# JulHoltzDevelopers/WavesAndEigenvalues.jl

Hardware: AMD Instinct MI355X
Metric: eigenpairs/sec (higher is better)
Workload: dtype f64

## Files before the change

### wavesandeigenvalues.jl_amd/csrc/beyn.hip

```cpp
#include <cmath>

#include "solver.h"

static void small_solve(std::vector<zc> &A, std::vector<zc> &b, int n) {
    std::vector<char> dead(n, 0);
    double amax = 0.0;
    for (const zc &a : A) amax = std::max(amax, std::abs(a));
    for (int k = 0; k < n; ++k) {
        int p = k;
        double best = 0.0;
        for (int i = k; i < n; ++i) { const double v = std::abs(A[(size_t)k * n + i]); if (v > best) { best = v; p = i; } }
        if (!(best > 1e-14 * amax)) { dead[k] = 1; continue; }
        if (p != k) {
            for (int j = 0; j < n; ++j) std::swap(A[(size_t)j * n + k], A[(size_t)j * n + p]);
            std::swap(b[k], b[p]);
        }
        const zc inv = 1.0 / A[(size_t)k * n + k];
        for (int i = k + 1; i < n; ++i) {
            const zc f = A[(size_t)k * n + i] * inv;
            if (f == zc(0)) continue;
            for (int j = k + 1; j < n; ++j) A[(size_t)j * n + i] -= f * A[(size_t)j * n + k];
            b[i] -= f * b[k];
        }
    }
    for (int k = n - 1; k >= 0; --k) {
        if (dead[k]) { b[k] = 0; continue; }
        zc sres = b[k];
        for (int j = k + 1; j < n; ++j) sres -= A[(size_t)j * n + k] * b[j];
        b[k] = sres / A[(size_t)k * n + k];
    }
}

static void rb_d2h(wae_family *h, const cplx *src, cplx *dst, size_t cnt) {
    HIP_CHECK(hipMemcpyAsync(dst, src, cnt * sizeof(cplx), hipMemcpyDeviceToHost, h->stream));
    HIP_CHECK(hipStreamSynchronize(h->stream));
}

static void rb_reset(wae_family *h, cplx *Q, int cap, int l, const double *table, int npts, const cplx *Vinter) {
    RbState &R = h->rb;
    const int T = h->T;
    R.Q = Q; R.cap = cap; R.l = l; R.S = 0;
    R.kact.clear();
    for (int k = 0; k < T; ++k) {
        bool used = false;
        for (int p = 0; p < npts && !used; ++p) used = table[((size_t)p * T + k) * 2] != 0.0 || table[((size_t)p * T + k) * 2 + 1] != 0.0;
        if (used) R.kact.push_back(k);
    }
    const size_t vecl = (size_t)h->d * l;
    R.wait_w();
    if (R.W.n < R.kact.size() * (size_t)cap * vecl) {
        const size_t need = R.kact.size() * (size_t)cap * vecl;
        const int dev = h->device;
        RbState *Rp = &R;
        R.w_job = std::async(std::launch::async, [Rp, need, dev]() {
            HIP_CHECK(hipSetDevice(dev));
            Rp->W.alloc(need);
        });
    }
    R.Hk.assign(R.kact.size() * (size_t)cap * cap * l, zc(0));
    R.g.assign((size_t)cap * l, zc(0));
    R.Vi.reserve(vecl);
    HIP_CHECK(hipMemcpyAsync(R.Vi.p, Vinter, vecl * sizeof(cplx), hipMemcpyDeviceToDevice, h->stream));
    R.vi_valid = true;
    R.hb.reserve((size_t)4 * (cap + 4) * l); R.alpha.reserve(l); R.alpha2.reserve((size_t)cap * l);
}

static void rb_append_block(wae_family *h, int cnt, const std::vector<std::vector<std::vector<zc>>> &pck) {
    RbState &R = h->rb;
    hipStream_t st = h->stream;
    const int64_t d = h->d;
    const int l = R.l, cap = R.cap, S = R.S;
    const size_t vecl = (size_t)d * l;
    std::vector<cplx> hh((size_t)(S + cnt) * cnt * l), n0((size_t)cnt * l), n1(l);
    const OpDev A0 = h->ops[0].dev(WAE_OP_N);
    cplx *qn = R.Q + (size_t)S * vecl;
    for (int j = 0; j < cnt; ++j) launch_norms(qn + (size_t)j * vecl, d, l, h->partial.p, R.hb.p + (size_t)j * l, st);
    rb_d2h(h, R.hb.p, n0.data(), (size_t)cnt * l);
    static const bool multi_axpy = !(getenv("WAE_RB_MULTI_AXPY") && atoi(getenv("WAE_RB_MULTI_AXPY")) == 0);
    const bool fits = (size_t)S * cnt * l * sizeof(cplx) <= 60 * 1024;
    for (int pass = 0; pass < 2 && S > 0; ++pass) {
        launch_dots_multi(R.Q, vecl, S, qn, vecl, cnt, d, l, h->partial.p, R.hb.p, st);
        if (multi_axpy && fits) {
            launch_axpy_neg_multi(R.Q, vecl, S, R.hb.p, qn, vecl, cnt, d, l, st);
            continue;
        }
        rb_d2h(h, R.hb.p, hh.data(), (size_t)S * cnt * l);
        std::vector<cplx> cj((size_t)S * l);
        for (int j = 0; j < cnt; ++j) {
            for (int i = 0; i < S; ++i)
                for (int c = 0; c < l; ++c) cj[(size_t)i * l + c] = hh[((size_t)i * cnt + j) * l + c];
            R.alpha2.upload(cj.data(), cj.size(), st);
            launch_axpy_neg(R.Q, vecl, S, R.alpha2.p, qn + (size_t)j * vecl, d, l, st);
            HIP_CHECK(hipStreamSynchronize(st));
        }
    }
    for (int j = 0; j < cnt; ++j) {
        cplx *q = qn + (size_t)j * vecl;
        for (int pass = 0; pass < 2 && j > 0; ++pass) {
            launch_dots(qn, vecl, j, q, d, l, h->partial.p, R.hb.p, st);
            launch_axpy_neg(qn, vecl, j, R.hb.p, q, d, l, st);
        }
        launch_norms(q, d, l, h->partial.p, R.hb.p, st);
        rb_d2h(h, R.hb.p, n1.data(), l);
        for (int c = 0; c < l; ++c) {
            const double nrm0 = n0[(size_t)j * l + c].x;
            n1[c] = (n1[c].x > 1e-9 * nrm0 && nrm0 > 0.0) ? cplx{n1[c].x, 0.0} : cplx{0.0, 0.0};
        }
        R.alpha.upload(n1.data(), l, st);
        launch_scale_inv(q, R.alpha.p, q, d, l, st);
        HIP_CHECK(hipStreamSynchronize(st));
    }
    launch_dots_multi(qn, vecl, cnt, R.Vi.p, vecl, 1, d, l, h->partial.p, R.hb.p, st);
    rb_d2h(h, R.hb.p, hh.data(), (size_t)cnt * l);
    for (int j = 0; j < cnt; ++j)
        for (int c = 0; c < l; ++c) R.g[(size_t)(S + j) * l + c] = zc(hh[(size_t)j * l + c].x, hh[(size_t)j * l + c].y);
    for (size_t ki = 0; ki < R.kact.size(); ++ki) {
        R.wait_w();
        cplx *Wk = R.W.p + ki * (size_t)cap * vecl;
        cplx *wn = Wk + (size_t)S * vecl;
        upload_pc(h, pck[ki]);
        for (int j = 0; j < cnt; ++j)
            launch_spmv(A0, pc_level(h, 0), l, qn + (size_t)j * vecl, wn + (size_t)j * vecl, nullptr, 0.0, l, MODE_AX, st);
        zc *H = &R.Hk[ki * (size_t)cap * cap * l];
        launch_dots_multi(R.Q, vecl, S + cnt, wn, vecl, cnt, d, l, h->partial.p, R.hb.p, st);
        rb_d2h(h, R.hb.p, hh.data(), (size_t)(S + cnt) * cnt * l);
        for (int i = 0; i < S + cnt; ++i)
            for (int j = 0; j < cnt; ++j)
                for (int c = 0; c < l; ++c) {
                    const cplx v = hh[((size_t)i * cnt + j) * l + c];
                    H[((size_t)(S + j) * cap + i) * l + c] = zc(v.x, v.y);
                }
        zc herm_factor(0);
        bool herm = false;
        {
            static const bool herm_on = !(getenv("WAE_RB_HERMITIAN") && atoi(getenv("WAE_RB_HERMITIAN")) == 0);
            const int kterm = R.kact[ki], pl = h->term_plane[kterm];
            const LevelOp &L0 = h->ops[0];
            for (size_t g = 0; g < L0.groups.size() && herm_on && !herm; ++g)
                for (int q = 0; q < L0.groups[g].nplanes; ++q)
                    if (h->slot_plane[0][(size_t)L0.groups[g].plane0 + q] == pl && L0.groups[g].symmetric && L0.groups[g].is_real) {
                        const zc sc = h->term_scale[kterm];
                        if (sc != zc(0)) { herm = true; herm_factor = sc / std::conj(sc); }
                    }
        }
        if (S > 0 && herm) {
            for (int i = 0; i < S; ++i)
                for (int j = 0; j < cnt; ++j)
                    for (int c = 0; c < l; ++c)
                        H[((size_t)i * cap + S + j) * l + c] = herm_factor * std::conj(H[((size_t)(S + j) * cap + i) * l + c]);
        } else if (S > 0) {
            launch_dots_multi(Wk, vecl, S, qn, vecl, cnt, d, l, h->partial.p, R.hb.p, st);
            rb_d2h(h, R.hb.p, hh.data(), (size_t)S * cnt * l);
            for (int i = 0; i < S; ++i)
                for (int j = 0; j < cnt; ++j)
                    for (int c = 0; c < l; ++c) {
                        const cplx v = hh[((size_t)i * cnt + j) * l + c];
                        H[((size_t)i * cap + S + j) * l + c] = zc(v.x, -v.y);
                    }
        }
    }
    R.S += cnt;
}

static void rb_append(wae_family *h, int count) {
    RbState &R = h->rb;
    WAE_REQUIRE(R.S + count <= R.cap, "snapshot store is full");
    std::vector<std::vector<std::vector<zc>>> pck(R.kact.size());
    for (size_t ki = 0; ki < R.kact.size(); ++ki) {
        std::vector<double> ek((size_t)2 * h->T, 0.0);
        ek[(size_t)2 * R.kact[ki]] = 1.0;
        pck[ki].resize(1);
        plane_coeffs(h, ek.data(), WAE_OP_N, pck[ki][0]);
    }
    for (int done = 0; done < count; done += 4) rb_append_block(h, std::min(4, count - done), pck);
}

static std::vector<cplx> rb_guess_coeffs(const wae_family *h, const double *ct_chunk, int ns) {
    const RbState &R = h->rb;
    const int S = R.S, l = R.l, cap = R.cap, T = h->T, nb = ns * l;
    std::vector<cplx> Y((size_t)S * nb);
    std::vector<zc> Hs((size_t)S * S), rhs(S);
    for (int sy = 0; sy < ns; ++sy) {
        const double *ct = ct_chunk + (size_t)sy * 2 * T;
        for (int k = 0; k < T; ++k)
            if ((ct[2 * k] != 0.0 || ct[2 * k + 1] != 0.0) && std::find(R.kact.begin(), R.kact.end(), k) == R.kact.end())
                throw WaeError(WAE_ERR_INVALID, "a term outside the projected set has a non-zero coefficient: rebuild the basis (mode 1)");
        for (int c = 0; c < l; ++c) {
            std::fill(Hs.begin(), Hs.end(), zc(0));
            for (size_t ki = 0; ki < R.kact.size(); ++ki) {
                const zc ck(ct[2 * R.kact[ki]], ct[2 * R.kact[ki] + 1]);
                if (ck == zc(0)) continue;
                const zc *H = &R.Hk[ki * (size_t)cap * cap * l];
                for (int sc = 0; sc < S; ++sc)
                    for (int i = 0; i < S; ++i) Hs[(size_t)sc * S + i] += ck * H[((size_t)sc * cap + i) * l + c];
            }
            for (int i = 0; i < S; ++i) rhs[i] = R.g[(size_t)i * l + c];
            small_solve(Hs, rhs, S);
            for (int i = 0; i < S; ++i) {
                const zc yv = std::isfinite(rhs[i].real()) && std::isfinite(rhs[i].imag()) ? rhs[i] : zc(0);
                Y[(size_t)i * nb + (size_t)sy * l + c] = cplx{yv.real(), yv.imag()};
            }
        }
    }
    return Y;
}
static void rb_apply_guess(wae_family *h, const std::vector<cplx> &Y, int ns, cplx *X) {
    RbState &R = h->rb;
    const int S = (int)(Y.size() / ((size_t)ns * R.l));
    R.ycoef.upload(Y.data(), Y.size(), h->stream);
    launch_lincomb_rep(R.Q, (size_t)h->d * R.l, S, R.ycoef.p, X, h->d, ns * R.l, R.l, h->stream);
    HIP_CHECK(hipStreamSynchronize(h->stream));
}

struct BeynPass {
    enum Keep { nothing, into_basis, raw_to_store };
    bool new_basis = false;
    int absorb = 0;
    bool solve = true;
    bool guess = false;
    Keep keep = nothing;
    int enrich_its = 1 << 30;
    bool light_cycle = false;
    bool progressive = false;
    bool prefetch_coeffs = false;
    int npts = 0;
    const double *z = nullptr, *w = nullptr, *coeff_table = nullptr;
    const double *V = nullptr;
    int l = 0, l_total = 0, col0 = 0;
    int K = 1, maxit = 0;
    double tol = 0.0;
    cplx *Q = nullptr;
    int nbasis = 0, slot0 = 0;
    double *A_out = nullptr;
    cplx *out_dev = nullptr;
    bool accumulate = false;
};

static BeynPass beyn_pass_for_mode(int mode, bool have_V, int npts, int nbasis, int slot0) {
    WAE_REQUIRE(have_V || mode == 2, "bad argument");
    WAE_REQUIRE(mode >= 0 && mode <= 4, "mode must be 0 (take snapshots), 1 (rebuild the basis from the store, use it), 2 (use it), "
                                        "3 (solve from zero, store raw) or 4 (build the basis from the store, solve nothing)");
    WAE_REQUIRE(nbasis >= 0 && slot0 >= 0 && (mode == 2 || slot0 + ((mode == 0 || mode == 3) ? npts : 0) <= nbasis), "snapshot slots out of range");
    static const int enrich_its = getenv("WAE_RB_ENRICH") ? atoi(getenv("WAE_RB_ENRICH")) : (1 << 30);
    BeynPass p;
// ... 40 lines not shown
    const bool store = p.new_basis || p.guess || p.keep != BeynPass::nothing;
    WAE_REQUIRE(!store || p.l <= h->NB, "l exceeds the solver batch width");
    HIP_CHECK(hipSetDevice(h->device));
    hipStream_t st = h->stream;
    CallInfo ci;
    const int64_t d = h->d;
    const int l = p.l, T = h->T, npts = p.npts, npow = 2 * p.K;
    const size_t acnt = (size_t)d * p.l_total * npow;
    const size_t vecl = (size_t)d * l;
    RbState &R = h->rb;
    DevBuf<cplx> Aown;
    cplx *Ad = p.out_dev;
    if (!Ad) { Aown.alloc(acnt); Ad = Aown.p; }
    if (!p.accumulate) launch_fill_zero(Ad, acnt, st);
    cplx *Q = p.Q;
    if (store && !Q) {
        if (p.new_basis && p.keep == BeynPass::into_basis) h->rbQ.reserve(vecl * (size_t)p.nbasis);
        WAE_REQUIRE(h->rbQ.n >= vecl * (size_t)p.nbasis, "no snapshots stored in the handle: run mode 0 first");
        Q = h->rbQ.p;
    }
    h->io_a.reserve(vecl);
    if (p.V) {
        HIP_CHECK(hipMemcpyAsync(h->io_a.p, p.V, vecl * sizeof(cplx), hipMemcpyHostToDevice, st));
    } else {
        WAE_REQUIRE(R.vi_valid && R.l == l && R.Vi.n >= vecl, "V may be NULL only in mode 2 after a mode 0/1 call with the same l on this handle");
        launch_inter_to_colmajor(R.Vi.p, l, d, l, h->io_a.p, st, h->perm());
    }
    if (p.guess) R.ycoef.reserve((size_t)std::max(p.nbasis, 1) * h->NB);
    if (p.new_basis) {
        launch_colmajor_to_inter(h->io_a.p, d, l, h->W.p, l, st, h->perm());
        rb_reset(h, Q, p.nbasis, l, p.coeff_table, npts, h->W.p);
        if (p.absorb > 0) rb_append(h, p.absorb);
    } else if (p.guess) {
        WAE_REQUIRE(R.Q == Q && R.l == l && R.cap == p.nbasis, "the basis in the handle belongs to another store / shape");
        WAE_REQUIRE(p.keep != BeynPass::into_basis || p.slot0 == R.S, "mode 0 appends: slot0 must equal the number of snapshots taken so far");
        WAE_REQUIRE(p.keep == BeynPass::into_basis || R.S > 0, "mode 2 needs a basis: run mode 0 (or 1) first");
    }
    if (!p.solve) {
        HIP_CHECK(hipStreamSynchronize(st));
        ci.li.levels = (int)h->ops.size();
        return ci.finish(info);
    }

    static const bool rbdbg = getenv("WAE_GMRES_DEBUG") && atoi(getenv("WAE_GMRES_DEBUG"));
    double t_guess = 0.0, t_solve = 0.0, t_append = 0.0;
    struct LightOff { bool &on; ~LightOff() { on = false; } } light_off{h->vc_light};
    for (int cg = 0; cg < l; cg += h->NB) {
        const int lg = std::min(h->NB, l - cg);
        const int spc = std::max(1, h->NB / lg);
        const int c0 = std::max(1, 16 / lg);
        h->zw_dev.reserve((size_t)2 * spc);
        std::future<std::vector<cplx>> next_Y;
        auto launch_coeffs = [&](int q0) {
            const int nq = std::min(spc, npts - q0);
            const double *ct = p.coeff_table + (size_t)q0 * 2 * T;
            return std::async(std::launch::async, [h, ct, nq]() { return rb_guess_coeffs(h, ct, nq); });
        };
        if (p.prefetch_coeffs && npts > 0 && R.S > 0) next_Y = launch_coeffs(0);
        int rep_nb = -1;
        for (int p0 = 0, ns; p0 < npts; p0 += ns) {
            ns = std::min(spc, npts - p0);
            if (p.progressive) ns = std::min(ns, std::max(c0, R.S));
            const Batch bt{ns * lg, lg, ns, WAE_OP_N};
            const auto pcs = beyn_chunk_prepare(h, p, p0, ns, cg, lg, rep_nb);
            const bool guess = p.guess && R.S > 0;
            const double ta = now_s();
            if (guess) {
                std::vector<cplx> Y;
                if (next_Y.valid()) {
                    Y = next_Y.get();
                    if (p0 + spc < npts) next_Y = launch_coeffs(p0 + spc);
                } else {
                    Y = rb_guess_coeffs(h, p.coeff_table + (size_t)p0 * 2 * T, ns);
                }
                rb_apply_guess(h, Y, ns, h->Xs.p);
            }
            const double tb = now_s();
// ... 52 lines not shown
        return beyn_pass_core(h, p, info);
    });
}

int wae_rb_export(wae_family *h, int32_t *S_out, int32_t *l_out, int32_t *nk_out, int32_t *kact_out, double *Hk_out, double *g_out) {
    return guarded([&]() {
        WAE_REQUIRE(h && S_out && l_out && nk_out, "bad argument");
        const RbState &R = h->rb;
        *S_out = R.S; *l_out = R.l; *nk_out = (int32_t)R.kact.size();
        if (kact_out) for (size_t i = 0; i < R.kact.size(); ++i) kact_out[i] = R.kact[i];
        const int S = R.S, l = R.l, cap = R.cap;
        if (Hk_out)
            for (size_t ki = 0; ki < R.kact.size(); ++ki)
                for (int s = 0; s < S; ++s)
                    for (int i = 0; i < S; ++i)
                        for (int c = 0; c < l; ++c) {
                            const zc v = R.Hk[ki * (size_t)cap * cap * l + ((size_t)s * cap + i) * l + c];
                            const size_t o = (((ki * S + s) * (size_t)S + i) * l + c) * 2;
                            Hk_out[o] = v.real(); Hk_out[o + 1] = v.imag();
                        }
        if (g_out)
            for (int i = 0; i < S; ++i)
                for (int c = 0; c < l; ++c) { g_out[((size_t)i * l + c) * 2] = R.g[(size_t)i * l + c].real(); g_out[((size_t)i * l + c) * 2 + 1] = R.g[(size_t)i * l + c].imag(); }
        return WAE_OK;
    });
}

int wae_rb_import(wae_family *h, int32_t S, int32_t l, uint64_t Q_dev, int32_t nk, const int32_t *kact, const double *Hk, const double *g) {
    return guarded([&]() {
        WAE_REQUIRE(h && S > 0 && l > 0 && Q_dev && nk >= 0 && (nk == 0 || kact) && Hk && g, "bad argument");
        RbState &R = h->rb;
        R.Q = (cplx *)(uintptr_t)Q_dev; R.cap = S; R.l = l; R.S = S;
        R.vi_valid = false;
        R.kact.assign(kact, kact + nk);
        R.Hk.resize((size_t)nk * S * S * l);
        for (size_t i = 0; i < R.Hk.size(); ++i) R.Hk[i] = zc(Hk[2 * i], Hk[2 * i + 1]);
        R.g.resize((size_t)S * l);
        for (size_t i = 0; i < R.g.size(); ++i) R.g[i] = zc(g[2 * i], g[2 * i + 1]);
        return WAE_OK;
    });
}

}
```

### wavesandeigenvalues.jl_amd/csrc/family.h

```cpp
#pragma once
#include <algorithm>
#include <chrono>
#include <future>

#include "amg.h"
#include "tiles.h"

struct RbState {
    cplx *Q = nullptr;
    int cap = 0, l = 0, S = 0;
    std::vector<int> kact;
    std::vector<zc> Hk;
    std::vector<zc> g;
    DevBuf<cplx> W, Vi, hb, alpha, alpha2, ycoef;
    std::future<void> w_job;
    void wait_w() { if (w_job.valid()) w_job.get(); }
    bool vi_valid = false;
    ~RbState() { if (w_job.valid()) w_job.wait(); }
};

struct wae_family {
    bool vc_light = false;
    int device = 0;
    hipStream_t stream = nullptr;
    int64_t d = 0;
    int T = 0;
    std::vector<int> term_plane;
    std::vector<zc> term_scale;
    std::vector<int64_t> term_nnz;
    int nplanes = 0;
    std::vector<CsrZ> planes0;
    std::vector<int> perm_h;
    DevBuf<int> perm_dev;
    std::vector<int> tile_row_ptr;
    const int *perm() const { return perm_dev.p; }
    std::vector<LevelOp> ops;
    std::vector<std::vector<int>> slot_plane;
    std::vector<Transfer> xfer;
    int64_t nc = 0;
    DevBuf<cplx> dense_planes, Ainv;
    DevBuf<int> dstatus;
    bool solver_ready = false;
    double jac_w = 0.8;
    double jac_w_post = 0.9;
    double jac_w_light = 0.5;
    int nsweeps = 1, restart = 30, NB = 64;
    std::vector<double> lvl_lambda, lvl_scale;
    std::vector<DevBuf<cplx>> lx, lb, lt;
    DevBuf<cplx> V, W, Z, Xs, Bs, U, partial, hdev, ydev, pcdev, one_dev, io_a, io_b, zw_dev;
    DevBuf<cplx> vsq;
    DevBuf<cplx> rbQ;
    RbState rb;
    DevBuf<int> plane_col_dev;
    DevBuf<unsigned char> cmask;
    DevBuf<cplx> gs_R, gs_sn, gs_g, gs_rescale, gs_Hraw, gs_pair;
    DevBuf<double> gs_sub;
    DevBuf<double> gs_cs, gs_sv, gs_relres, gs_bnorm, gs_hist;
    DevBuf<int> gs_int;
    DevBuf<unsigned char> gs_done;
    int64_t n_penalty = 0;
    LevelOp pen_op;
    std::vector<int> pen_slot;
    LevelOp pen_row_op;
    std::vector<int> pen_row_slot;
    DevBuf<int> pen_rows;
    DevBuf<cplx> pen_b, pen_x, pen_t;
    struct Slot { DevBuf<cplx> buf; int ncols = 0; };
    Slot slots[WAE_NSLOTS];
    DevBuf<cplx> arn_EV, arn_t, arn_pcM, arn_hcol, arn_stage, arn_gdir;
    int arn_nsys = 0, arn_cols = 0;
    DevBuf<cplx> pt_ws;
    DevBuf<cplx> pt_Gd, pt_pcd;
    cplx *h_pinned = nullptr;
    cplx *h_pin_pair = nullptr;
    size_t h_pin_pair_n = 0;
    size_t pc_stride_level = 0;
    ~wae_family() {
        if (stream) (void)hipStreamSynchronize(stream);
        if (h_pinned) (void)hipHostFree(h_pinned);
        if (h_pin_pair) (void)hipHostFree(h_pin_pair);
        if (stream) (void)hipStreamDestroy(stream);
    }
};

struct Batch {
// ... 26 lines not shown
```

### wavesandeigenvalues.jl_amd/csrc/setup.hip

```cpp
#include <atomic>
#include <cmath>
#include <exception>
#include <limits>
#include <map>
#include <memory>
#include <tuple>

#include "family.h"

OpDev LevelOp::dev(int op) const {
    OpDev o;
    memset(&o, 0, sizeof(o));
    o.ngroups = (int)groups.size();
    o.nplanes_total = nplanes;
    o.n = n;
    o.diag = diag.p;
    o.conj_diag = (op == WAE_OP_C) ? 1 : 0;
    o.tiles = !tiles.ready ? nullptr : (op == WAE_OP_N || tiles.all_symmetric) ? &tiles.dev : (tiles.ready_t ? &tiles.dev_t : nullptr);
    {
        const LongRows &LR = (op == WAE_OP_N) ? long_n : long_t;
        o.nlong = LR.n;
        o.long_rows = LR.rows.p; o.long_ptr = LR.ptr.p; o.long_col = LR.col.p; o.long_slot = LR.slot.p;
        o.long_val = LR.val.p; o.long_acc = LR.acc.p; o.long_part = LR.part.p;
        o.long_conj = (op == WAE_OP_C) ? 1 : 0;
// ... 727 lines not shown
        lap("permutation");
        const bool with_tiles = !row_ptr.empty();
        auto xj = std::async(std::launch::async, [&, h, with_tiles]() {
            HIP_CHECK(hipSetDevice(h->device));
            const OwnStream s2;
            upload_transfer(xfer0, L0, s2.s);
            if (with_tiles && env.tile_restrict) build_restriction_tiles(xfer0, L0.R, TILE_WCAP_COARSE, s2.s, env.debug);
            if (!h->tile_row_ptr.empty() && env.xfer_tiles) build_transfer_tiles(xfer0, L0.P, h->tile_row_ptr, s2.s);
        });
        const std::vector<CsrZ> &pl1 = planes.empty() ? L0.coarse_planes : planes;
        slot_plane = build_levelop(op, pl1, s3.s, WAE_LEVEL_SYM_TOL, env);
        lap("operator groups");
        if (with_tiles) build_level_tiles(op, pl1, slot_plane, row_ptr, s3.s, env, 4);
        HIP_CHECK(hipStreamSynchronize(s3.s));
        lap("tile storage");
        xj.get();
        lap("wait for the transfer");
        built = true;
        seconds = now_s() - tq0;
    }
};

template <class ColMap> static CsrZ extract_rows(const CsrZ &A, const std::vector<int> &rows, int64_t m, ColMap &&col_of) {
    CsrZ B;
    B.n = (int64_t)rows.size();
    B.m = m;
    B.ptr.assign(rows.size() + 1, 0);
    for (size_t i = 0; i < rows.size(); ++i) {
        for (int pp = A.ptr[rows[i]]; pp < A.ptr[rows[i] + 1]; ++pp)
            if (col_of(A.col[pp]) >= 0) { B.col.push_back(col_of(A.col[pp])); B.val.push_back(A.val[pp]); }
        B.ptr[i + 1] = (int)B.col.size();
    }
    return B;
}

static std::vector<CsrD> read_prolongators(int64_t d, int32_t nlev, const int64_t *rows, const int64_t *cols, const int32_t *const *ptr,
                                           const int32_t *const *col, const double *const *val) {
    WAE_REQUIRE(nlev >= 1, "nested set-up: nlev must be at least 1");
    WAE_REQUIRE(rows && cols && ptr && col && val, "nested set-up: a null array");
    std::vector<CsrD> Ps((size_t)nlev);
    for (int32_t k = 0; k < nlev; ++k) {
        const std::string at = " (prolongator " + std::to_string(k) + ")";
        WAE_REQUIRE(ptr[k] && col[k] && val[k], "nested set-up: a null array" + at);
        if (k == 0) WAE_REQUIRE(rows[0] == d, "nested set-up: prolongator 0 has " + std::to_string(rows[0]) + " rows, the family has " + std::to_string(d) + " unknowns");
        else WAE_REQUIRE(rows[k] == cols[k - 1], "nested set-up: the dimensions do not chain: " + std::to_string(rows[k]) + " rows after " + std::to_string(cols[k - 1]) + " columns" + at);
        WAE_REQUIRE(cols[k] >= 1 && cols[k] < 2147483647 && rows[k] >= 1, "nested set-up: bad dimensions" + at);
        CsrD &P = Ps[(size_t)k];
        P.n = rows[k]; P.m = cols[k];
        const int32_t *pp = ptr[k];
        WAE_REQUIRE(pp[0] == 0, "nested set-up: the row pointer does not start at 0" + at);
        for (int64_t i = 0; i < P.n; ++i) WAE_REQUIRE(pp[i] <= pp[i + 1], "nested set-up: the row pointer is not monotone" + at);
        const int64_t nnz = pp[P.n];
        P.ptr.assign(pp, pp + P.n + 1);
        P.col.assign(col[k], col[k] + nnz);
        P.val.assign(val[k], val[k] + nnz);
        for (int64_t i = 0; i < P.n; ++i)
            for (int e = P.ptr[i]; e < P.ptr[i + 1]; ++e) {
                WAE_REQUIRE(P.col[e] >= 0 && P.col[e] < P.m, "nested set-up: a column out of range" + at);
                WAE_REQUIRE(e == P.ptr[i] || P.col[e - 1] < P.col[e], "nested set-up: unsorted or duplicate columns in a row" + at);
                WAE_REQUIRE(std::isfinite(P.val[e]), "nested set-up: a value that is not finite" + at);
            }
    }
    return Ps;
}
static CsrD take_rows_drop_columns(const CsrD &P, const std::vector<int> &src, std::vector<int> &kept) {
    CsrD B;
// ... 418 lines not shown
```

### wavesandeigenvalues.jl_amd/csrc/solver.h

```cpp
#pragma once
#include "family.h"

void upload_pc(wae_family *h, const std::vector<std::vector<zc>> &pcs);
const cplx *pc_level(const wae_family *h, int l);
void dense_setup(wae_family *h, const Batch &bt);
double pre_weight(const wae_family *h, int l = 0);
struct CycleNorms { cplx *out; bool only; bool done = false; };
cplx *vcycle(wae_family *h, const Batch &bt, int l, const cplx *b, const unsigned char *cm = nullptr, bool have_x0 = false,
             cplx *final_out = nullptr, CycleNorms *cn = nullptr);
void penalty_polish(wae_family *h, const Batch &bt, const cplx *B, cplx *X);
int gmres(wae_family *h, const Batch &bt, const cplx *B, cplx *X, double tol, int maxit, wae_solve_info *info, const cplx *guess_dir = nullptr,
          bool have_x0 = false, double *relres_out = nullptr);
int solve_chunk(wae_family *h, const Batch &bt, const std::vector<std::vector<zc>> &pcs, const cplx *B, cplx *X, double tol, int maxit,
                wae_solve_info *info, const cplx *guess_dir = nullptr, bool have_x0 = false);
struct CallInfo {
    wae_solve_info li{};
    double t0 = now_s();
    int finish(wae_solve_info *out);
};

cplx *slot_col(wae_family *h, int32_t slot, int32_t col);
const cplx *slot_cols_ptr(wae_family *h, int32_t slot, const int32_t *cols, int n, DevBuf<cplx> &stage, hipStream_t st);
```

### wavesandeigenvalues.jl_amd/csrc/vec.hip

```cpp
#include <type_traits>

#include "block_reduce.h"
#include "kernel_helpers.h"

__global__ void fill_zero_kernel(cplx *X, size_t count) {
    for (size_t e = (size_t)blockIdx.x * 256 + threadIdx.x; e < count; e += (size_t)gridDim.x * 256) X[e] = cplx{0.0, 0.0};
}
void launch_fill_zero(cplx *X, size_t count, hipStream_t st) {
    if (!count) return;
    hipLaunchKernelGGL(fill_zero_kernel, dim3(grid_for(count)), dim3(256), 0, st, X, count);
    HIP_CHECK(hipGetLastError());
}
void launch_copy(const cplx *X, cplx *Y, size_t count, hipStream_t st) {
    if (!count) return;
    HIP_CHECK(hipMemcpyAsync(Y, X, count * sizeof(cplx), hipMemcpyDeviceToDevice, st));
}
__global__ void add_kernel(const cplx *__restrict__ X, cplx *__restrict__ Y, size_t count) {
    for (size_t e = (size_t)blockIdx.x * 256 + threadIdx.x; e < count; e += (size_t)gridDim.x * 256) {
        cplx a = X[e], b = Y[e];
        Y[e] = cplx{a.x + b.x, a.y + b.y};
    }
}
void launch_add(const cplx *X, cplx *Y, size_t count, hipStream_t st) {
    if (!count) return;
// ... 114 lines not shown
            cplx w[NW];
#pragma unroll
            for (int j = 0; j < NW; ++j) w[j] = j < nw ? W[(size_t)j * sw + e] : cplx{0.0, 0.0};
#pragma unroll
            for (int i = 0; i < MAXV; ++i) {
                if (i < nv) {
                    const cplx v = V[(size_t)i * sv + e];
#pragma unroll
                    for (int j = 0; j < NW; ++j) {
                        acc[i][j].x += v.x * w[j].x + v.y * w[j].y;
                        acc[i][j].y += v.x * w[j].y - v.y * w[j].x;
                    }
                }
            }
        }
    }
#pragma unroll
    for (int i = 0; i < MAXV; ++i) {
#pragma unroll
        for (int j = 0; j < NW; ++j) {
            if (i < nv && j < nw) {
                const cplx s = block_colsum<false, 256>(acc[i][j], nb, sm);
                if (tid < nb) partial[((size_t)blockIdx.x * nv * nw + (size_t)i * nw + j) * nb + tid] = s;
            }
        }
    }
}
void launch_dots_multi(const cplx *V, size_t sv, int nv, const cplx *W, size_t sw, int nw, int64_t n, int nb, cplx *partial, cplx *out,
                       hipStream_t st) {
    if (nb < 1 || nb > 256 || nw < 1 || nw > 4) throw WaeError(WAE_ERR_INVALID, "dots_multi: nb in 1..256, nw in 1..4");
    int done = 0;
    while (done < nv) {
        const int chunk = std::min(8, nv - done);
        const int nblk = 768;
        hipLaunchKernelGGL((dots_multi_kernel<8, 4>), dim3(nblk), dim3(256), 0, st, V + (size_t)done * sv, sv, chunk, W, sw, nw, n, nb, partial);
        HIP_CHECK(hipGetLastError());
        const int count = chunk * nw * nb;
        launch_reduce_partials(partial, nblk, count, out + (size_t)done * nw * nb, 0, st);
        done += chunk;
    }
}
void launch_dots(const cplx *V, size_t stride, int nv, const cplx *W, int64_t n, int nb, cplx *partial, cplx *out, hipStream_t st,
                 const unsigned char *cmask) {
    dots_impl(V, stride, nv, W, n, nb, partial, out, 0, st, cmask);
}
void launch_dots_scaled(const cplx *V, size_t stride, int nv, const cplx *W, int64_t n, int nb, cplx *partial, cplx *out, const cplx *scale,
                        hipStream_t st, const unsigned char *cmask) {
    dots_impl(V, stride, nv, W, n, nb, partial, out, 0, st, cmask, scale);
}
void launch_norms(const cplx *X, int64_t n, int nb, cplx *partial, cplx *out, hipStream_t st, const unsigned char *cmask) {
    dots_impl(X, 0, 1, X, n, nb, partial, out, 1, st, cmask);
}

constexpr int AXU = 8;
constexpr int AX_MAXC = 4096;
__device__ __forceinline__ bool nonzero(const cplx &c) { return c.x != 0.0 || c.y != 0.0; }
template <bool NORM>
__global__ __launch_bounds__(256) void axpy_neg_kernel(const cplx *__restrict__ V, size_t stride, int nv, const cplx *__restrict__ h,
                                                       cplx *W, int64_t n, int nb, double sign, const cplx *base,
                                                       const unsigned char *__restrict__ cmask, cplx *__restrict__ partial) {
    extern __shared__ cplx hs[];
    const int tid = threadIdx.x;
    for (int k = tid; k < nv * nb; k += 256) {
        const cplx c = h[k];
        hs[k] = cplx{sign * c.x, sign * c.y};
    }
    __syncthreads();
    const int R = 256 / nb;
    const int b = tid % nb, rl = tid / nb;
    const bool live = rl < R && !(cmask && !cmask[b >> 3]);
    if (!NORM && !live) return;
// ... 892 lines not shown
```

### wavesandeigenvalues.jl_amd/csrc/wae_internal.h

```cpp
#pragma once
#include <hip/hip_runtime.h>
#include <algorithm>
#include <cmath>
#include <complex>
#include <cstdint>
#include <cstdio>
#include <cstring>
#include <new>
#include <stdexcept>
#include <string>
#include <vector>

#include "../../include/waehip.h"

typedef std::complex<double> zc;
typedef double2 cplx;

struct WaeError : std::runtime_error {
    int code;
    WaeError(int c, const std::string &m) : std::runtime_error(m), code(c) {}
};
void wae_set_error(const std::string &m);
int wae_internal_device(const wae_family *h);
hipStream_t wae_internal_stream(const wae_family *h);
// ... 273 lines not shown
void launch_dense_assemble(const cplx *planes, int nplanes, int n, const cplx *pc, int nsys, int op,
                           cplx *Ainv, hipStream_t s);
void launch_dense_invert(cplx *Ainv, int n, int nsys, int *status, hipStream_t s);
void launch_dense_apply(const cplx *Ainv, int n, int cps, const cplx *X, cplx *Y, int nb, hipStream_t s, const unsigned char *cmask = nullptr);

void launch_fill_zero(cplx *X, size_t count, hipStream_t s);
void launch_copy(const cplx *X, cplx *Y, size_t count, hipStream_t s);
void launch_dots(const cplx *V, size_t stride, int nv, const cplx *W, int64_t n, int nb, cplx *partial, cplx *out, hipStream_t s,
                 const unsigned char *cmask = nullptr);
void launch_axpy_neg_multi(const cplx *V, size_t stride, int nv, const cplx *h, cplx *W, size_t wstride, int cnt, int64_t n, int nb, hipStream_t s);
void launch_axpy_neg(const cplx *V, size_t stride, int nv, const cplx *h, cplx *W, int64_t n, int nb, hipStream_t s,
                     const unsigned char *cmask = nullptr);
void launch_axpy_neg_norm(const cplx *V, size_t stride, int nv, const cplx *h, cplx *W, int64_t n, int nb, cplx *partial, cplx *norms,
                          hipStream_t s, const unsigned char *cmask = nullptr, const cplx *base = nullptr, cplx *inv_out = nullptr);
void launch_dots_scaled(const cplx *V, size_t stride, int nv, const cplx *W, int64_t n, int nb, cplx *partial, cplx *out, const cplx *scale,
                        hipStream_t s, const unsigned char *cmask = nullptr);
void launch_lincomb(const cplx *V, size_t stride, int nv, const cplx *y, cplx *Y, int64_t n, int nb, hipStream_t s);
void launch_lincomb_add(const cplx *V, size_t stride, int nv, const cplx *y, cplx *X, int64_t n, int nb, hipStream_t s);
void launch_norms(const cplx *X, int64_t n, int nb, cplx *partial, cplx *out, hipStream_t s, const unsigned char *cmask = nullptr);
void launch_scale_inv(const cplx *X, const cplx *alpha, cplx *Y, int64_t n, int nb, hipStream_t s, const unsigned char *cmask = nullptr);
void launch_axpby1(cplx a, const cplx *x, cplx b, const cplx *y, cplx *out, size_t n, hipStream_t s, int conj_x = 0);
void launch_add(const cplx *X, cplx *Y, size_t count, hipStream_t s);
void launch_colmajor_to_inter(const cplx *Xc, int64_t d, int r, cplx *Xi, int nb, hipStream_t s, const int *perm = nullptr);
void launch_inter_to_colmajor(const cplx *Xi, int nb, int64_t d, int r, cplx *Xc, hipStream_t s, const int *perm = nullptr);
void launch_replicate(const cplx *Vc, int64_t d, int l, cplx *Xi, int nb, hipStream_t s, const int *perm = nullptr);
constexpr int PROLONG_NORM_BLOCKS = 1024;
void launch_prolong_add(const int *ptr, const int *col, const double *val, int64_t n, const cplx *Xc, const cplx *X, cplx *Y, int nb, hipStream_t s,
                        const unsigned char *cmask = nullptr, cplx *partial = nullptr, cplx *norms = nullptr);
void launch_reduce_partials(const cplx *partial, int nblk, int count, cplx *out, int do_sqrt, hipStream_t s, const cplx *scale = nullptr,
                            cplx *inv_out = nullptr);
void launch_dots_multi(const cplx *V, size_t sv, int nv, const cplx *W, size_t sw, int nw, int64_t n, int nb, cplx *partial, cplx *out,
                       hipStream_t s);
void launch_gather_rows(const cplx *X, const int *rows, int64_t nrows, int nb, cplx *out, hipStream_t s);
void launch_scatter_add_rows(const cplx *D, const int *rows, int64_t nrows, int nb, cplx *X, hipStream_t s);
void launch_extract_cols(const cplx *X, int nb, int off, int l, cplx *out, int64_t n, hipStream_t s);
void launch_lincomb_rep(const cplx *Q, size_t stride, int nv, const cplx *y, cplx *X, int64_t n, int nb, int l, hipStream_t s);
void launch_mask_cols(cplx *X, const cplx *keep, int64_t n, int nb, hipStream_t s);
void launch_beyn_accum(const cplx *Xi, int nb, int64_t d, int l, int nsys, const cplx *w, const cplx *z, int npow, cplx *A, hipStream_t s,
                       int lA = 0, int c0 = 0, const int *perm = nullptr);
void launch_pt_gemm_batch(const cplx *V, size_t stride, int k, const cplx *G, cplx *U, int64_t d, int T, int nb, hipStream_t s);
void launch_pt_spmv_batch(const OpDev &op, const cplx *pc, const int *plane_col, const cplx *U, int nin, cplx *Y, int nb, int accumulate,
                          hipStream_t s);
void launch_pt_axpby_cols(const cplx *coef, const cplx *x, const cplx *y, cplx *out, int64_t d, int nb, hipStream_t s);
void launch_pt_project(cplx *vk, const cplx *v0, const cplx *dots, int nd, int64_t d, int nb, hipStream_t s);
struct GmresDev {
    int nb, m, histcap;
    cplx *R;
    double *cs;
    cplx *sn;
    cplx *g;
    double *sv;
    cplx *vsq;
    int *conv, *steps, *iters, *histlen, *stalled;
    double *relres, *bnorm;
    double *hist;
    cplx *rescale;
    int *status;
    unsigned char *cmask;
    cplx *Hraw;
    double *sub;
};
void launch_gmres_init(const GmresDev &S, const cplx *beta, const unsigned char *done, int use_mask, hipStream_t s);
void launch_gmres_step(const GmresDev &S, const cplx *hd, int j, double tol, double lim, int use_mask, cplx *Vnew, int64_t n, hipStream_t s,
                       const cplx *rn = nullptr);
void launch_dots2_scaled(const cplx *V, size_t stride, int nv, const cplx *W1, const cplx *W2, int64_t n, int nb, cplx *partial, cplx *out1,
                         cplx *out2, cplx *gram_out, const cplx *scale, hipStream_t s, const unsigned char *cmask = nullptr);
// ... 8 lines not shown
```

Baseline: 4.417.

## Restrict reduced-basis projections to sparse term support rows and grow basis in place

```diff
diff --git a/wavesandeigenvalues.jl_amd/csrc/beyn.hip b/wavesandeigenvalues.jl_amd/csrc/beyn.hip
--- a/wavesandeigenvalues.jl_amd/csrc/beyn.hip
+++ b/wavesandeigenvalues.jl_amd/csrc/beyn.hip
@@ -36,6 +36,68 @@
     HIP_CHECK(hipStreamSynchronize(h->stream));
 }
 
+static bool rb_debug() {
+    static const bool on = getenv("WAE_GMRES_DEBUG") && atoi(getenv("WAE_GMRES_DEBUG"));
+    return on;
+}
+
+static bool rb_term_hermitian(const wae_family *h, int kterm, zc &factor) {
+    static const bool herm_on = !(getenv("WAE_RB_HERMITIAN") && atoi(getenv("WAE_RB_HERMITIAN")) == 0);
+    const int pl = h->term_plane[kterm];
+    const LevelOp &L0 = h->ops[0];
+    const zc sc = h->term_scale[kterm];
+    factor = zc(0);
+    if (!herm_on || sc == zc(0)) return false;
+    for (size_t g = 0; g < L0.groups.size(); ++g)
+        for (int q = 0; q < L0.groups[g].nplanes; ++q)
+            if (h->slot_plane[0][(size_t)L0.groups[g].plane0 + q] == pl && L0.groups[g].symmetric && L0.groups[g].is_real) {
+                factor = sc / std::conj(sc);
+                return true;
+            }
+    return false;
+}
+
+static void rb_setup(wae_family *h, const cplx *Vinter) {
+    RbState &R = h->rb;
+    const int cap = R.cap, l = R.l;
+    const size_t vecl = (size_t)h->d * l;
+    R.wait_w();
+    static const bool support_on = !(getenv("WAE_RB_SUPPORT") && atoi(getenv("WAE_RB_SUPPORT")) == 0);
+    if (R.term.size() != R.kact.size()) { R.term.clear(); R.term.resize(R.kact.size()); }
+    size_t nres = 0;
+    for (size_t ki = 0; ki < R.kact.size(); ++ki) {
+        RbState::Term &t = R.term[ki];
+        const int k = R.kact[ki];
+        t.herm = rb_term_hermitian(h, k, t.herm_factor);
+        const RbSupport &sup = term_support(h, k, l);
+        t.sup = support_on && sup.sparse ? &sup : nullptr;
+        t.resident = !t.sup && !t.herm;
+        t.woff = t.resident ? nres++ * (size_t)cap * vecl : 0;
+        if (t.sup) t.Qs.reserve((size_t)cap * sup.n * l); else t.Qs.release();
+        if (t.sup && !t.herm) t.Ws.reserve((size_t)cap * sup.n * l); else t.Ws.release();
+        if (rb_debug())
+            fprintf(stderr, "[rb] term %d: %lld support rows of %lld, %s path%s\n", k, (long long)sup.n, (long long)h->d, t.sup ? "support" : "dense",
+                    t.herm ? ", Hermitian rows" : "");
+    }
+    R.wn.reserve((size_t)4 * vecl);
+    size_t nsup = 0;
+    for (const RbState::Term &t : R.term) if (t.sup) nsup = std::max(nsup, (size_t)t.sup->n);
+    R.wc.reserve((size_t)4 * nsup * l);
+    if (R.W.n < nres * (size_t)cap * vecl) {
+        const size_t need = nres * (size_t)cap * vecl;
+        const int dev = h->device;
+        RbState *Rp = &R;
+        R.w_job = std::async(std::launch::async, [Rp, need, dev]() {
+            HIP_CHECK(hipSetDevice(dev));
+            Rp->W.alloc(need);
+        });
+    }
+    R.Vi.reserve(vecl);
+    HIP_CHECK(hipMemcpyAsync(R.Vi.p, Vinter, vecl * sizeof(cplx), hipMemcpyDeviceToDevice, h->stream));
+    R.vi_valid = true;
+    R.hb.reserve((size_t)4 * (cap + 4) * l); R.alpha.reserve(l); R.alpha2.reserve((size_t)cap * l);
+}
+
 static void rb_reset(wae_family *h, cplx *Q, int cap, int l, const double *table, int npts, const cplx *Vinter) {
     RbState &R = h->rb;
     const int T = h->T;
@@ -46,23 +108,55 @@
         for (int p = 0; p < npts && !used; ++p) used = table[((size_t)p * T + k) * 2] != 0.0 || table[((size_t)p * T + k) * 2 + 1] != 0.0;
         if (used) R.kact.push_back(k);
     }
-    const size_t vecl = (size_t)h->d * l;
-    R.wait_w();
-    if (R.W.n < R.kact.size() * (size_t)cap * vecl) {
-        const size_t need = R.kact.size() * (size_t)cap * vecl;
-        const int dev = h->device;
-        RbState *Rp = &R;
-        R.w_job = std::async(std::launch::async, [Rp, need, dev]() {
-            HIP_CHECK(hipSetDevice(dev));
-            Rp->W.alloc(need);
-        });
-    }
+    rb_setup(h, Vinter);
     R.Hk.assign(R.kact.size() * (size_t)cap * cap * l, zc(0));
     R.g.assign((size_t)cap * l, zc(0));
-    R.Vi.reserve(vecl);
-    HIP_CHECK(hipMemcpyAsync(R.Vi.p, Vinter, vecl * sizeof(cplx), hipMemcpyDeviceToDevice, h->stream));
-    R.vi_valid = true;
-    R.hb.reserve((size_t)4 * (cap + 4) * l); R.alpha.reserve(l); R.alpha2.reserve((size_t)cap * l);
+}
+
+static std::vector<std::vector<std::vector<zc>>> rb_term_coeffs(const wae_family *h) {
+    const RbState &R = h->rb;
+    std::vector<std::vector<std::vector<zc>>> pck(R.kact.size());
+    for (size_t ki = 0; ki < R.kact.size(); ++ki) {
+        std::vector<double> ek((size_t)2 * h->T, 0.0);
+        ek[(size_t)2 * R.kact[ki]] = 1.0;
+        pck[ki].resize(1);
+        plane_coeffs(h, ek.data(), WAE_OP_N, pck[ki][0]);
+    }
+    return pck;
+}
+
+static void rb_grow(wae_family *h, int newcap, const cplx *Vinter) {
+    RbState &R = h->rb;
+    hipStream_t st = h->stream;
+    const int S = R.S, l = R.l, oc = R.cap;
+    const size_t vecl = (size_t)h->d * l;
+    std::vector<zc> Hn(R.kact.size() * (size_t)newcap * newcap * l, zc(0));
+    for (size_t ki = 0; ki < R.kact.size(); ++ki)
+        for (int s = 0; s < S; ++s)
+            for (int i = 0; i < S; ++i)
+                for (int c = 0; c < l; ++c)
+                    Hn[ki * (size_t)newcap * newcap * l + ((size_t)s * newcap + i) * l + c] = R.Hk[ki * (size_t)oc * oc * l + ((size_t)s * oc + i) * l + c];
+    R.Hk.swap(Hn);
+    R.g.resize((size_t)newcap * l, zc(0));
+    R.cap = newcap;
+    rb_setup(h, Vinter);
+    const auto pck = rb_term_coeffs(h);
+    const OpDev A0 = h->ops[0].dev(WAE_OP_N);
+    for (size_t ki = 0; ki < R.kact.size(); ++ki) {
+        RbState::Term &t = R.term[ki];
+        const size_t vl = (size_t)(t.sup ? t.sup->n : h->d) * l;
+        if (t.sup)
+            for (int s = 0; s < S; ++s) launch_gather_rows(R.Q + (size_t)s * vecl, t.sup->rows.p, t.sup->n, l, t.Qs.p + (size_t)s * vl, st);
+        if (t.herm) continue;
+        if (t.resident) R.wait_w();
+        upload_pc(h, pck[ki]);
+        cplx *Wk = t.sup ? t.Ws.p : R.W.p + t.woff;
+        for (int s = 0; s < S; ++s) {
+            launch_spmv(A0, pc_level(h, 0), l, R.Q + (size_t)s * vecl, t.sup ? R.wn.p : Wk + (size_t)s * vl, nullptr, 0.0, l, MODE_AX, st);
+            if (t.sup) launch_gather_rows(R.wn.p, t.sup->rows.p, t.sup->n, l, Wk + (size_t)s * vl, st);
+        }
+    }
+    HIP_CHECK(hipStreamSynchronize(st));
 }
 
 static void rb_append_block(wae_family *h, int cnt, const std::vector<std::vector<std::vector<zc>>> &pck) {
@@ -108,6 +202,8 @@
         }
         R.alpha.upload(n1.data(), l, st);
         launch_scale_inv(q, R.alpha.p, q, d, l, st);
+        for (RbState::Term &t : R.term)
+            if (t.sup) launch_gather_rows(q, t.sup->rows.p, t.sup->n, l, t.Qs.p + (size_t)(S + j) * t.sup->n * l, st);
         HIP_CHECK(hipStreamSynchronize(st));
     }
     launch_dots_multi(qn, vecl, cnt, R.Vi.p, vecl, 1, d, l, h->partial.p, R.hb.p, st);
@@ -115,14 +211,23 @@
     for (int j = 0; j < cnt; ++j)
         for (int c = 0; c < l; ++c) R.g[(size_t)(S + j) * l + c] = zc(hh[(size_t)j * l + c].x, hh[(size_t)j * l + c].y);
     for (size_t ki = 0; ki < R.kact.size(); ++ki) {
-        R.wait_w();
-        cplx *Wk = R.W.p + ki * (size_t)cap * vecl;
-        cplx *wn = Wk + (size_t)S * vecl;
+        RbState::Term &t = R.term[ki];
+        const int64_t nr = t.sup ? t.sup->n : d;
+        const size_t vl = (size_t)nr * l;
+        const cplx *Qk = t.sup ? t.Qs.p : R.Q;
+        const cplx *qk = Qk + (size_t)S * vl;
+        cplx *Wk = nullptr;
+        if (t.sup && !t.herm) Wk = t.Ws.p;
+        if (t.resident) { R.wait_w(); Wk = R.W.p + t.woff; }
+        cplx *wn = Wk ? Wk + (size_t)S * vl : (t.sup ? R.wc.p : R.wn.p);
         upload_pc(h, pck[ki]);
-        for (int j = 0; j < cnt; ++j)
-            launch_spmv(A0, pc_level(h, 0), l, qn + (size_t)j * vecl, wn + (size_t)j * vecl, nullptr, 0.0, l, MODE_AX, st);
+        for (int j = 0; j < cnt; ++j) {
+            launch_spmv(A0, pc_level(h, 0), l, qn + (size_t)j * vecl, t.sup ? R.wn.p : wn + (size_t)j * vl, nullptr, 0.0, l, MODE_AX, st);
+            if (t.sup) launch_gather_rows(R.wn.p, t.sup->rows.p, t.sup->n, l, wn + (size_t)j * vl, st);
+        }
         zc *H = &R.Hk[ki * (size_t)cap * cap * l];
-        launch_dots_multi(R.Q, vecl, S + cnt, wn, vecl, cnt, d, l, h->partial.p, R.hb.p, st);
+        if (t.sup) launch_dots_multi_rows(Qk, vl, S + cnt, wn, vl, cnt, t.sup->tptr.p, l, h->partial.p, R.hb.p, st);
+        else launch_dots_multi(Qk, vl, S + cnt, wn, vl, cnt, nr, l, h->partial.p, R.hb.p, st);
         rb_d2h(h, R.hb.p, hh.data(), (size_t)(S + cnt) * cnt * l);
         for (int i = 0; i < S + cnt; ++i)
             for (int j = 0; j < cnt; ++j)
@@ -130,26 +235,14 @@
                     const cplx v = hh[((size_t)i * cnt + j) * l + c];
                     H[((size_t)(S + j) * cap + i) * l + c] = zc(v.x, v.y);
                 }
-        zc herm_factor(0);
-        bool herm = false;
-        {
-            static const bool herm_on = !(getenv("WAE_RB_HERMITIAN") && atoi(getenv("WAE_RB_HERMITIAN")) == 0);
-            const int kterm = R.kact[ki], pl = h->term_plane[kterm];
-            const LevelOp &L0 = h->ops[0];
-            for (size_t g = 0; g < L0.groups.size() && herm_on && !herm; ++g)
-                for (int q = 0; q < L0.groups[g].nplanes; ++q)
-                    if (h->slot_plane[0][(size_t)L0.groups[g].plane0 + q] == pl && L0.groups[g].symmetric && L0.groups[g].is_real) {
-                        const zc sc = h->term_scale[kterm];
-                        if (sc != zc(0)) { herm = true; herm_factor = sc / std::conj(sc); }
-                    }
-        }
-        if (S > 0 && herm) {
+        if (S > 0 && t.herm) {
             for (int i = 0; i < S; ++i)
                 for (int j = 0; j < cnt; ++j)
                     for (int c = 0; c < l; ++c)
-                        H[((size_t)i * cap + S + j) * l + c] = herm_factor * std::conj(H[((size_t)(S + j) * cap + i) * l + c]);
+                        H[((size_t)i * cap + S + j) * l + c] = t.herm_factor * std::conj(H[((size_t)(S + j) * cap + i) * l + c]);
         } else if (S > 0) {
-            launch_dots_multi(Wk, vecl, S, qn, vecl, cnt, d, l, h->partial.p, R.hb.p, st);
+            if (t.sup) launch_dots_multi_rows(Wk, vl, S, qk, vl, cnt, t.sup->tptr.p, l, h->partial.p, R.hb.p, st);
+            else launch_dots_multi(Wk, vl, S, qk, vl, cnt, nr, l, h->partial.p, R.hb.p, st);
             rb_d2h(h, R.hb.p, hh.data(), (size_t)S * cnt * l);
             for (int i = 0; i < S; ++i)
                 for (int j = 0; j < cnt; ++j)
@@ -165,13 +258,7 @@
 static void rb_append(wae_family *h, int count) {
     RbState &R = h->rb;
     WAE_REQUIRE(R.S + count <= R.cap, "snapshot store is full");
-    std::vector<std::vector<std::vector<zc>>> pck(R.kact.size());
-    for (size_t ki = 0; ki < R.kact.size(); ++ki) {
-        std::vector<double> ek((size_t)2 * h->T, 0.0);
-        ek[(size_t)2 * R.kact[ki]] = 1.0;
-        pck[ki].resize(1);
-        plane_coeffs(h, ek.data(), WAE_OP_N, pck[ki][0]);
-    }
+    const auto pck = rb_term_coeffs(h);
     for (int done = 0; done < count; done += 4) rb_append_block(h, std::min(4, count - done), pck);
 }
 
@@ -207,9 +294,19 @@
 static void rb_apply_guess(wae_family *h, const std::vector<cplx> &Y, int ns, cplx *X) {
     RbState &R = h->rb;
     const int S = (int)(Y.size() / ((size_t)ns * R.l));
-    R.ycoef.upload(Y.data(), Y.size(), h->stream);
+    if (R.ypin_n < Y.size()) {
+        HIP_CHECK(hipStreamSynchronize(h->stream));
+        const size_t n = std::max(Y.size(), (size_t)std::max(R.cap, 1) * h->NB);
+        if (R.ypin) HIP_CHECK(hipHostFree(R.ypin));
+        R.ypin = nullptr; R.ypin_n = 0;
+        HIP_CHECK(hipHostMalloc((void **)&R.ypin, n * sizeof(cplx)));
+        R.ypin_n = n;
+    }
+    cplx *pin = R.ypin;
+    std::copy(Y.begin(), Y.end(), pin);
+    R.ycoef.reserve(Y.size());
+    HIP_CHECK(hipMemcpyAsync(R.ycoef.p, pin, Y.size() * sizeof(cplx), hipMemcpyHostToDevice, h->stream));
     launch_lincomb_rep(R.Q, (size_t)h->d * R.l, S, R.ycoef.p, X, h->d, ns * R.l, R.l, h->stream);
-    HIP_CHECK(hipStreamSynchronize(h->stream));
 }
 
 struct BeynPass {
@@ -316,6 +413,10 @@
         rb_reset(h, Q, p.nbasis, l, p.coeff_table, npts, h->W.p);
         if (p.absorb > 0) rb_append(h, p.absorb);
     } else if (p.guess) {
+        if (p.keep == BeynPass::into_basis && R.Q == Q && R.l == l && R.S == R.cap && !R.vi_valid && p.nbasis > R.cap && p.slot0 == R.S) {
+            launch_colmajor_to_inter(h->io_a.p, d, l, h->W.p, l, st, h->perm());
+            rb_grow(h, p.nbasis, h->W.p);
+        }
         WAE_REQUIRE(R.Q == Q && R.l == l && R.cap == p.nbasis, "the basis in the handle belongs to another store / shape");
         WAE_REQUIRE(p.keep != BeynPass::into_basis || p.slot0 == R.S, "mode 0 appends: slot0 must equal the number of snapshots taken so far");
         WAE_REQUIRE(p.keep == BeynPass::into_basis || R.S > 0, "mode 2 needs a basis: run mode 0 (or 1) first");
@@ -326,7 +427,7 @@
         return ci.finish(info);
     }
 
-    static const bool rbdbg = getenv("WAE_GMRES_DEBUG") && atoi(getenv("WAE_GMRES_DEBUG"));
+    const bool rbdbg = rb_debug();
     double t_guess = 0.0, t_solve = 0.0, t_append = 0.0;
     struct LightOff { bool &on; ~LightOff() { on = false; } } light_off{h->vc_light};
     for (int cg = 0; cg < l; cg += h->NB) {
@@ -445,6 +546,7 @@
         RbState &R = h->rb;
         R.Q = (cplx *)(uintptr_t)Q_dev; R.cap = S; R.l = l; R.S = S;
         R.vi_valid = false;
+        R.term.clear();
         R.kact.assign(kact, kact + nk);
         R.Hk.resize((size_t)nk * S * S * l);
         for (size_t i = 0; i < R.Hk.size(); ++i) R.Hk[i] = zc(Hk[2 * i], Hk[2 * i + 1]);
diff --git a/wavesandeigenvalues.jl_amd/csrc/family.h b/wavesandeigenvalues.jl_amd/csrc/family.h
--- a/wavesandeigenvalues.jl_amd/csrc/family.h
+++ b/wavesandeigenvalues.jl_amd/csrc/family.h
@@ -6,17 +6,39 @@
 #include "amg.h"
 #include "tiles.h"
 
+struct RbSupport {
+    bool built = false, sparse = false;
+    int l = 0;
+    int64_t n = 0;
+    DevBuf<int> rows;
+    DevBuf<int> tptr;
+};
+
 struct RbState {
     cplx *Q = nullptr;
     int cap = 0, l = 0, S = 0;
     std::vector<int> kact;
     std::vector<zc> Hk;
     std::vector<zc> g;
-    DevBuf<cplx> W, Vi, hb, alpha, alpha2, ycoef;
+    struct Term {
+        bool herm = false;
+        zc herm_factor{0.0, 0.0};
+        const RbSupport *sup = nullptr;
+        DevBuf<cplx> Qs, Ws;
+        size_t woff = 0;
+        bool resident = false;
+    };
+    std::vector<Term> term;
+    DevBuf<cplx> W, wn, wc, Vi, hb, alpha, alpha2, ycoef;
     std::future<void> w_job;
     void wait_w() { if (w_job.valid()) w_job.get(); }
     bool vi_valid = false;
-    ~RbState() { if (w_job.valid()) w_job.wait(); }
+    cplx *ypin = nullptr;
+    size_t ypin_n = 0;
+    ~RbState() {
+        if (w_job.valid()) w_job.wait();
+        if (ypin) (void)hipHostFree(ypin);
+    }
 };
 
 struct wae_family {
@@ -51,6 +73,7 @@
     DevBuf<cplx> vsq;
     DevBuf<cplx> rbQ;
     RbState rb;
+    std::vector<RbSupport> rb_sup;
     DevBuf<int> plane_col_dev;
     DevBuf<unsigned char> cmask;
     DevBuf<cplx> gs_R, gs_sn, gs_g, gs_rescale, gs_Hraw, gs_pair;
diff --git a/wavesandeigenvalues.jl_amd/csrc/setup.hip b/wavesandeigenvalues.jl_amd/csrc/setup.hip
--- a/wavesandeigenvalues.jl_amd/csrc/setup.hip
+++ b/wavesandeigenvalues.jl_amd/csrc/setup.hip
@@ -783,6 +783,33 @@
         B.ptr[i + 1] = (int)B.col.size();
     }
     return B;
+}
+
+const RbSupport &term_support(wae_family *h, int k, int l) {
+    if (h->rb_sup.empty()) h->rb_sup.resize((size_t)h->T);
+    RbSupport &sup = h->rb_sup[(size_t)k];
+    if (sup.built && sup.l == l) return sup;
+    const CsrZ &A = h->planes0[(size_t)h->term_plane[(size_t)k]];
+    std::vector<int> rows;
+    for (int64_t i = 0; i < A.n; ++i)
+        if (A.ptr[i + 1] > A.ptr[i]) rows.push_back((int)i);
+    sup.n = (int64_t)rows.size();
+    sup.sparse = sup.n > 0 && sup.n * 8 <= A.n && l >= 1 && l <= 256;
+    sup.l = l;
+    if (sup.sparse) {
+        const int R = 256 / l;
+        auto owner = [R](int row) { return (int64_t)((row / R) % DOTS_MULTI_BLOCKS) * R + row % R; };
+        std::stable_sort(rows.begin(), rows.end(), [&](int a, int b) { return owner(a) < owner(b); });
+        std::vector<int> tptr((size_t)DOTS_MULTI_BLOCKS * R + 1, 0);
+        for (int r : rows) ++tptr[(size_t)owner(r) + 1];
+        for (size_t i = 1; i < tptr.size(); ++i) tptr[i] += tptr[i - 1];
+        hipStream_t st = h->stream;
+        sup.rows.upload(rows.data(), rows.size(), st);
+        sup.tptr.upload(tptr.data(), tptr.size(), st);
+        HIP_CHECK(hipStreamSynchronize(st));
+    }
+    sup.built = true;
+    return sup;
 }
 
 static std::vector<CsrD> read_prolongators(int64_t d, int32_t nlev, const int64_t *rows, const int64_t *cols, const int32_t *const *ptr,
diff --git a/wavesandeigenvalues.jl_amd/csrc/solver.h b/wavesandeigenvalues.jl_amd/csrc/solver.h
--- a/wavesandeigenvalues.jl_amd/csrc/solver.h
+++ b/wavesandeigenvalues.jl_amd/csrc/solver.h
@@ -19,5 +19,7 @@
     int finish(wae_solve_info *out);
 };
 
+const RbSupport &term_support(wae_family *h, int k, int l);
+
 cplx *slot_col(wae_family *h, int32_t slot, int32_t col);
 const cplx *slot_cols_ptr(wae_family *h, int32_t slot, const int32_t *cols, int n, DevBuf<cplx> &stage, hipStream_t st);
diff --git a/wavesandeigenvalues.jl_amd/csrc/vec.hip b/wavesandeigenvalues.jl_amd/csrc/vec.hip
--- a/wavesandeigenvalues.jl_amd/csrc/vec.hip
+++ b/wavesandeigenvalues.jl_amd/csrc/vec.hip
@@ -170,11 +170,67 @@
     int done = 0;
     while (done < nv) {
         const int chunk = std::min(8, nv - done);
-        const int nblk = 768;
+        const int nblk = DOTS_MULTI_BLOCKS;
         hipLaunchKernelGGL((dots_multi_kernel<8, 4>), dim3(nblk), dim3(256), 0, st, V + (size_t)done * sv, sv, chunk, W, sw, nw, n, nb, partial);
         HIP_CHECK(hipGetLastError());
         const int count = chunk * nw * nb;
         launch_reduce_partials(partial, nblk, count, out + (size_t)done * nw * nb, 0, st);
+        done += chunk;
+    }
+}
+template <int MAXV, int NW>
+__global__ __launch_bounds__(256) void dots_multi_rows_kernel(const cplx *__restrict__ V, size_t sv, int nv, const cplx *__restrict__ W, size_t sw, int nw,
+                                                              const int *__restrict__ tptr, int nb, cplx *__restrict__ partial) {
+    __shared__ cplx sm[256];
+    const int tid = threadIdx.x;
+    const int R = 256 / nb;
+    const int b = tid % nb, rl = tid / nb;
+    cplx acc[MAXV][NW];
+#pragma unroll
+    for (int i = 0; i < MAXV; ++i)
+#pragma unroll
+        for (int j = 0; j < NW; ++j) acc[i][j] = cplx{0.0, 0.0};
+    if (rl < R) {
+        const int p1 = tptr[(size_t)blockIdx.x * R + rl + 1];
+        for (int pos = tptr[(size_t)blockIdx.x * R + rl]; pos < p1; ++pos) {
+            const size_t e = (size_t)pos * nb + b;
+            cplx w[NW];
+#pragma unroll
+            for (int j = 0; j < NW; ++j) w[j] = j < nw ? W[(size_t)j * sw + e] : cplx{0.0, 0.0};
+#pragma unroll
+            for (int i = 0; i < MAXV; ++i) {
+                if (i < nv) {
+                    const cplx v = V[(size_t)i * sv + e];
+#pragma unroll
+                    for (int j = 0; j < NW; ++j) {
+                        acc[i][j].x += v.x * w[j].x + v.y * w[j].y;
+                        acc[i][j].y += v.x * w[j].y - v.y * w[j].x;
+                    }
+                }
+            }
+        }
+    }
+#pragma unroll
+    for (int i = 0; i < MAXV; ++i) {
+#pragma unroll
+        for (int j = 0; j < NW; ++j) {
+            if (i < nv && j < nw) {
+                const cplx s = block_colsum<false, 256>(acc[i][j], nb, sm);
+                if (tid < nb) partial[((size_t)blockIdx.x * nv * nw + (size_t)i * nw + j) * nb + tid] = s;
+            }
+        }
+    }
+}
+void launch_dots_multi_rows(const cplx *V, size_t sv, int nv, const cplx *W, size_t sw, int nw, const int *tptr, int nb, cplx *partial, cplx *out,
+                            hipStream_t st) {
+    if (nb < 1 || nb > 256 || nw < 1 || nw > 4) throw WaeError(WAE_ERR_INVALID, "dots_multi_rows: nb in 1..256, nw in 1..4");
+    int done = 0;
+    while (done < nv) {
+        const int chunk = std::min(8, nv - done);
+        const int nblk = DOTS_MULTI_BLOCKS;
+        hipLaunchKernelGGL((dots_multi_rows_kernel<8, 4>), dim3(nblk), dim3(256), 0, st, V + (size_t)done * sv, sv, chunk, W, sw, nw, tptr, nb, partial);
+        HIP_CHECK(hipGetLastError());
+        launch_reduce_partials(partial, nblk, chunk * nw * nb, out + (size_t)done * nw * nb, 0, st);
         done += chunk;
     }
 }
diff --git a/wavesandeigenvalues.jl_amd/csrc/wae_internal.h b/wavesandeigenvalues.jl_amd/csrc/wae_internal.h
--- a/wavesandeigenvalues.jl_amd/csrc/wae_internal.h
+++ b/wavesandeigenvalues.jl_amd/csrc/wae_internal.h
@@ -329,6 +329,9 @@
 void launch_dots_multi(const cplx *V, size_t sv, int nv, const cplx *W, size_t sw, int nw, int64_t n, int nb, cplx *partial, cplx *out,
                        hipStream_t s);
 void launch_gather_rows(const cplx *X, const int *rows, int64_t nrows, int nb, cplx *out, hipStream_t s);
+constexpr int DOTS_MULTI_BLOCKS = 768;
+void launch_dots_multi_rows(const cplx *V, size_t sv, int nv, const cplx *W, size_t sw, int nw, const int *tptr, int nb, cplx *partial, cplx *out,
+                            hipStream_t s);
 void launch_scatter_add_rows(const cplx *D, const int *rows, int64_t nrows, int nb, cplx *X, hipStream_t s);
 void launch_extract_cols(const cplx *X, int nb, int off, int l, cplx *out, int64_t n, hipStream_t s);
 void launch_lincomb_rep(const cplx *Q, size_t stride, int nv, const cplx *y, cplx *X, int64_t n, int nb, int l, hipStream_t s);
```

Result: no change. 4.455, median of 6 (+0.9%).
